# kkromberg/SpeechRecognition

Measured on AMD Instinct MI355X. Metric: frames/sec scored+decoded, higher is better.
Workload: dtype f64

## Files before the change

speechrecognition_amd/build.py:

```python
from __future__ import annotations

import hashlib
import os
import subprocess
import sys

HERE = os.path.dirname(os.path.abspath(__file__))
CSRC = os.path.join(HERE, "csrc")
LIB = os.path.join(HERE, "libsrgpu.so")
SOURCES = ["srgpu_api.cpp", "mixset.cpp", "feeder.cpp", "gmm_mfma.hip", "gmm_exact.hip", "gmm_prefilter.hip", "viterbi_decode.hip",
           "viterbi_fast.hip", "viterbi_words.hip", "viterbi_align.hip", "viterbi_fb.hip", "viterbi_netfb.hip", "viterbi_mmi.hip", "viterbi_smbr.hip", "viterbi_lattice.hip", "viterbi_bigram.hip", "viterbi_bigram_fb.hip", "viterbi_bigram_mmi.hip", "viterbi_bigram_lattice.hip",
           "em_accumulate.hip", "em_finalize.hip", "fmllr_stats.hip", "fmllr.cpp"]
HEADERS = ["kernels.h", "host_util.h", "handles.h", "traceback.h", "dpp_util.h", "netfb_device.h", os.path.join("..", "..", "include", "srgpu.h")]
FLAGS = ["-O3", "-std=c++17", "--offload-arch=gfx950", "-fPIC", "-fvisibility=hidden", "-Wall", "-Wno-unused-function"]
PER_FILE = {"gmm_exact.hip": ["-ffp-contract=off"], "gmm_prefilter.hip": ["-ffp-contract=off"], "em_accumulate.hip": ["-ffp-contract=off"],
            "em_finalize.hip": ["-ffp-contract=off"],
            "viterbi_bigram_lattice.hip": ["-ffp-contract=off"],
            "fmllr_stats.hip": ["-ffp-contract=off"]}
MAX_PARALLEL = 8


def _read(path):
    with open(path, "rb") as f:
        return f.read()


def _stamp_of(parts):
    h = hashlib.sha256()
    for p in parts:
        h.update(len(p).to_bytes(8, "little"))
        h.update(p)
    return h.hexdigest()


def _stored(path):
    try:
# ... 102 lines not shown
```

speechrecognition_amd/csrc/gmm_prefilter.hip:

```cpp
#include <hip/hip_runtime.h>
#include <stdint.h>

#include <algorithm>
#include <cmath>
#include <vector>

#include "kernels.h"

#ifndef SR_P16_NB
#define SR_P16_NB 4
#endif

namespace srgpu {

typedef float v4f __attribute__((ext_vector_type(4)));
static constexpr int kPWaves = 4;
static constexpr int kGroupBlocks = 8;

typedef _Float16 f16x8 __attribute__((ext_vector_type(8)));

__device__ inline uint32_t pack_f16x2(_Float16 l, _Float16 h) {
  return (uint32_t)__builtin_bit_cast(uint16_t, l) | ((uint32_t)__builtin_bit_cast(uint16_t, h) << 16);
}

template <int KS32, int NB>
__global__ __launch_bounds__(kPWaves * 64, (NB <= 2 ? 3 : 2)) void gmm_prefilter16_kernel(GmmPrefilterArgs a) {
  constexpr int kBlockBytes = KS32 * 1024;
  constexpr int kStageBytes = kGroupBlocks * kBlockBytes;
  constexpr int kChunksPerStage = kStageBytes / 1024;
  constexpr int kDmaPerWave = kChunksPerStage / kPWaves;
// ... 284 lines not shown
    case 4: hipLaunchKernelGGL((gmm_prefilter16_kernel<4, SR_P16_NB>), grid, block, 0, stream, a); break;
    default: return hipErrorInvalidValue;
  }
  return hipGetLastError();
}
int gmm_prefilter_frames_per_tile() { return kPWaves * SR_P16_NB * 16; }

#pragma clang fp contract(off)

#ifndef SR_R_THREADS
#define SR_R_THREADS 768
#endif
#ifndef SR_R_BATCH
#define SR_R_BATCH 4
#endif
static constexpr int kRThreads = SR_R_THREADS;
static constexpr int kRThreadsWide = 512;
static constexpr int kRWaves = kRThreads / 64;
static constexpr int kRBatch = SR_R_BATCH;
#ifndef SR_R_BATCH_WIDE
#define SR_R_BATCH_WIDE 8
#endif
static constexpr int kRBatchWide = SR_R_BATCH_WIDE;
static constexpr uint32_t kRingEntries = 128;
static constexpr uint32_t kRingLists = 2 * 8 * kRingEntries;
static constexpr uint32_t kRingWave = 4 * kRingLists;
struct __attribute__((aligned(16))) RingEntry { uint32_t lf, mask; double score; };
struct __attribute__((packed, aligned(4))) RowPiece { float v[4]; };

template <int DT, int NS, int SPW, int CH, int NT = kRThreads, int VS = 1, bool DEFER = false>
__global__ __launch_bounds__(NT) void gmm_refine_kernel(GmmRefineArgs a) {
  static_assert(DT > 0 && (DT & 1), "padded dimension: odd");
  static_assert(!DEFER || CH > 1, "deferred lists: states of several chunks");
  constexpr int kRThreads = NT, kRWaves = NT / 64;
  static_assert(CH == 1 || CH == 2 || CH == 4, "chunks per state (half)");
  static_assert(VS == 1 || (VS == 2 && CH == 4), "two halves only of four-chunk states");
  static_assert(SPW % (CH * VS) == 0 && (CH == 1 || SPW % 4 == 0), "a state's chunks live in one workgroup");
  extern __shared__ __attribute__((aligned(1024))) unsigned char panel_raw[];
  const uint32_t D = (uint32_t)DT, tid = threadIdx.x;
  const int lane = tid & 63, wave = tid >> 6;
  const uint32_t s0 = blockIdx.x * SPW;
  const uint32_t ns = (s0 + SPW <= a.n_pstates) ? SPW : a.n_pstates - s0;
  const uint32_t state_bytes = (2u * D + 2u) * NS * 8u;
  const uint64_t f_begin = (uint64_t)blockIdx.y * a.frames_per_split;
  const uint64_t f_end = (f_begin + a.frames_per_split < a.n_frames) ? f_begin + a.frames_per_split : a.n_frames;

  {
    const uint32_t chunks = (ns * state_bytes + 1023u) >> 10;
    const unsigned char* src = reinterpret_cast<const unsigned char*>(a.rows) + (uint64_t)s0 * state_bytes + lane * 16;
    for (uint32_t ch = wave; ch < chunks; ch += kRWaves)
// ... 10 lines not shown
  uint32_t n_eval = 0;
  double x[DT];
  const __amdgpu_buffer_rsrc_t featsT_rsrc = __builtin_amdgcn_make_buffer_rsrc(
      const_cast<float*>(a.featsT), 0, (int)0xFFFFFFFFu, 0x00020000);
  const uint32_t ld4 = (uint32_t)a.n_frames_ld * 4u;
  auto load_x = [&](uint64_t f) __attribute__((always_inline)) {
    const uint32_t voff = (uint32_t)f * 4u;
#pragma unroll
    for (int k = 0; k < DT; k++)
      x[k] = (double)__builtin_bit_cast(float, __builtin_amdgcn_raw_buffer_load_b32(featsT_rsrc, voff, (uint32_t)k * ld4, 0));
  };
  auto load_x_row = [&](uint64_t f) __attribute__((always_inline)) {
    const float* xr = a.feats + f * (uint64_t)DT;
#pragma unroll
    for (int q = 0; q < DT / 4; q++) {
      const RowPiece t = reinterpret_cast<const RowPiece*>(xr)[q];
#pragma unroll
      for (int i = 0; i < 4; i++) x[4 * q + i] = (double)t.v[i];
    }
#pragma unroll
    for (int k = DT - DT % 4; k < DT; k++) x[k] = (double)xr[k];
  };
  auto evaluate = [&](const unsigned char* col0) __attribute__((always_inline)) -> double {
    const volatile __attribute__((address_space(3))) double* col =
        (const volatile __attribute__((address_space(3))) double*)col0;
    double l0 = 0.0, l1 = 0.0, dist, score;
    {
      constexpr int RB = NT == kRThreadsWide ? kRBatchWide : kRBatch;
      constexpr int NB_ = (DT + 1 + RB - 1) / RB;
      double pm[2][RB], pv[2][RB];
#pragma unroll
      for (int i = 0; i < RB; i++)
        if (i <= DT) { pm[0][i] = col[(2 * i) * NS]; pv[0][i] = col[(2 * i + 1) * NS]; }
#pragma unroll
      for (int b = 0; b < NB_; b++) {
        const int cur = b & 1;
        __builtin_amdgcn_sched_barrier(0);
#pragma unroll
        for (int i = 0; i < RB; i++) {
          const int k = (b + 1) * RB + i;
          if (k <= DT) { pm[cur ^ 1][i] = col[(2 * k) * NS]; pv[cur ^ 1][i] = col[(2 * k + 1) * NS]; }
        }
        __builtin_amdgcn_sched_barrier(0);
#pragma unroll
        for (int i = 0; i < RB; i++) {
          const int k = b * RB + i;
          if (k < (int)(DT - (DT & 1))) {
            double u = x[k] - pm[cur][i];
            u = u * u;
            u = u * pv[cur][i];
            if (k & 1) l1 = l1 + u; else l0 = l0 + u;
          } else if (k == DT - 1) {
            dist = l0 + l1;
            const double t = x[k] - pm[cur][i];
            dist += t * t * pv[cur][i];
          } else if (k == DT) {
            if (!(DT & 1)) dist = l0 + l1;
            score = pm[cur][i] + dist / 2;
            score -= pv[cur][i];
          }
        }
        asm volatile("" : "+v"(l0), "+v"(l1));
      }
    }
// ... 22 lines not shown

  const uint32_t n_it = (uint32_t)((f_end - f_begin + kRThreads - 1) / kRThreads);
  for (uint32_t it = 0; it < n_it; it++) {
    const uint64_t fr = f_wave + (uint64_t)it * kRThreads + lane;
    const bool valid = fr < f_end;
    const uint64_t f = valid ? fr : f_end - 1;
    const uint32_t lf = it * 64u + (uint32_t)lane;
    load_x(f);
    constexpr int RS = SPW / (CH * VS);
    double res[RS];
    if constexpr (CH == 1) {
#pragma unroll
      for (int h = 0; h < SPW / 4; h++) {
        const uint4 v = reinterpret_cast<const uint4*>(a.mask)[(uint64_t)((s0 >> 2) + h) * a.n_frames + f];
        const uint32_t mk[4] = {v.x, v.y, v.z, v.w};
#pragma unroll
        for (int jj = 0; jj < 4; jj++) {
          const int j = 4 * h + jj;
          const uint32_t n = nd[j];
          uint32_t mask = mk[jj];
          mask &= n >= 32 ? 0xFFFFFFFFu : ((1u << n) - 1u);
          res[j] = 1e10;
          if (n) {
            const double score = evaluate(panel_raw + (size_t)j * state_bytes + (uint32_t)__builtin_ctz(mask | 0x80000000u) * 8u);
            res[j] = mask != 0 ? seeded_min(score) : res[j];
            if (counting) n_eval += (uint32_t)__builtin_popcountll(__ballot(valid));
          }
          const bool more = valid && (mask & (mask - 1)) != 0;
          const uint64_t b = __ballot(more);
          if (b) {
            const uint32_t c1 = (uint32_t)(cnt1 >> (8 * j)) & 0xFFu;
            const uint32_t pos = c1 + __builtin_amdgcn_mbcnt_hi((uint32_t)(b >> 32), __builtin_amdgcn_mbcnt_lo((uint32_t)b, 0u));
            if (more) {
              ring[(uint32_t)j * kRingEntries + pos] = RingEntry{lf, mask & (mask - 1), res[j]};
            }
            cnt1 += (uint64_t)__builtin_popcountll(b) << (8 * j);
          }
        }
      }
      if (valid) {
        if (a.chunks == 1) {
          double* o = a.out + f * a.ld + s0;
          if (ns == SPW) {
#pragma unroll
            for (int j = 0; j < SPW; j += 2) *reinterpret_cast<double2*>(o + j) = make_double2(res[j], res[j + 1]);
          } else {
#pragma unroll
// ... 12 lines not shown
#pragma unroll
          for (int j = 0; j < SPW; j += 4) {
            double m = res[j + 1] < res[j] ? res[j + 1] : res[j];
            m = res[j + 2] < m ? res[j + 2] : m;
            m = res[j + 3] < m ? res[j + 3] : m;
            if ((uint32_t)j < ns) o[j / 4] = m;
          }
        }
      }
    } else {
      auto append = [&](int j, bool more, uint32_t rest, double& best) __attribute__((always_inline)) {
        const uint64_t b = __ballot(more);
        if (b) {
          if constexpr (DEFER) {
            const uint32_t nb = (uint32_t)__builtin_popcountll(b);
            if (dcnt[DEFER ? j : 0] + nb <= a.defer_cap) {
              const uint32_t pos = dcnt[DEFER ? j : 0] + __builtin_amdgcn_mbcnt_hi((uint32_t)(b >> 32), __builtin_amdgcn_mbcnt_lo((uint32_t)b, 0u));
              if (more) seg[(uint64_t)j * a.defer_cap + pos] = RingEntry{(uint32_t)f, rest, best};
              dcnt[DEFER ? j : 0] += nb;
            } else {
              uint32_t mm = more ? rest : 0u;
              const unsigned char* panel = panel_raw + (size_t)j * state_bytes;
              do {
                const double score = evaluate(panel + (uint32_t)__builtin_ctz(mm | 0x80000000u) * 8u);
                if (counting) n_eval += (uint32_t)__builtin_popcountll(__ballot(mm != 0));
                if (mm != 0 && score < best) best = score;
                mm &= mm - 1;
              } while (__any(mm != 0));
            }
          } else {
          const uint32_t c1 = (uint32_t)(cnt1 >> (8 * j)) & 0xFFu;
          const uint32_t pos = c1 + __builtin_amdgcn_mbcnt_hi((uint32_t)(b >> 32), __builtin_amdgcn_mbcnt_lo((uint32_t)b, 0u));
          if (more) {
            ring[(uint32_t)j * kRingEntries + pos] = RingEntry{lf, rest, best};
          }
          cnt1 += (uint64_t)__builtin_popcountll(b) << (8 * j);
          }
        }
      };
      uint32_t mk[SPW];
#pragma unroll
      for (int h = 0; h < SPW / 4; h++) {
        const uint4 v = reinterpret_cast<const uint4*>(a.mask)[(uint64_t)((s0 >> 2) + h) * a.n_frames + f];
        mk[4 * h] = v.x; mk[4 * h + 1] = v.y; mk[4 * h + 2] = v.z; mk[4 * h + 3] = v.w;
      }
#pragma unroll
      for (int j = 0; j < SPW; j++) mk[j] &= nd[j] >= 32 ? 0xFFFFFFFFu : ((1u << nd[j]) - 1u);
      if constexpr (VS == 1) {
#pragma unroll
      for (int r = 0; r < RS; r++) {
        uint32_t msel = mk[r * CH], off = 0;
#pragma unroll
        for (int c = 1; c < CH; c++) {
          const bool empty = msel == 0;
          msel = empty ? mk[r * CH + c] : msel;
          off = empty ? (uint32_t)c * state_bytes : off;
        }
        res[r] = 1e10;
        if (nd[r * CH]) {
          const double score = evaluate(panel_raw + (size_t)(r * CH) * state_bytes + off + (uint32_t)__builtin_ctz(msel | 0x80000000u) * 8u);
          res[r] = msel != 0 ? seeded_min(score) : res[r];
          if (counting) n_eval += (uint32_t)__builtin_popcountll(__ballot(valid));
        }
#pragma unroll
        for (int c = 0; c < CH; c++) {
          const bool is_sel = off == (uint32_t)c * state_bytes;
          const uint32_t rest = is_sel ? msel & (msel - 1) : mk[r * CH + c];
          if (nd[r * CH + c]) append(r * CH + c, valid && rest != 0, rest, res[r]);
        }
      }
      } else {
#pragma unroll
      for (int r = 0; r < RS; r++) res[r] = 1e10;
#pragma unroll
      for (int rv = 0; rv < RS * VS; rv++) {
        uint32_t msel = mk[rv * CH], off = 0;
#pragma unroll
        for (int c = 1; c < CH; c++) {
          const bool empty = msel == 0;
          msel = empty ? mk[rv * CH + c] : msel;
          off = empty ? (uint32_t)c * state_bytes : off;
        }
        double resv = 1e10;
        if (nd[rv * CH]) {
          const double score = evaluate(panel_raw + (size_t)(rv * CH) * state_bytes + off + (uint32_t)__builtin_ctz(msel | 0x80000000u) * 8u);
          resv = msel != 0 ? seeded_min(score) : resv;
          if (counting) n_eval += (uint32_t)__builtin_popcountll(__ballot(valid));
        }
        if constexpr (VS == 1) res[rv] = resv;
        else res[rv / VS] = resv < res[rv / VS] ? resv : res[rv / VS];
#pragma unroll
        for (int c = 0; c < CH; c++) {
          const bool is_sel = off == (uint32_t)c * state_bytes;
          const uint32_t rest = is_sel ? msel & (msel - 1) : mk[rv * CH + c];
          if (nd[rv * CH + c]) append(rv * CH + c, valid && rest != 0, rest, resv);
        }
        if constexpr (DEFER && VS == 2) res[rv / VS] = resv < res[rv / VS] ? resv : res[rv / VS];
      }
      }
      if (valid) {
        double* o = a.out + f * a.ld + s0 / (CH * VS);
        if (ns == SPW && RS >= 2) {
#pragma unroll
          for (int r = 0; r + 1 < RS; r += 2) *reinterpret_cast<double2*>(o + r) = make_double2(res[r], res[r + 1]);
        } else {
#pragma unroll
          for (int r = 0; r < RS; r++)
            if ((uint32_t)(r * CH * VS) < ns) o[r] = res[r];
// ... 19 lines not shown
      const bool l1 = level == 1;
      const uint32_t have = (uint32_t)((l1 ? cnt1 : cnt2) >> (8u * j)) & 0xFFu;
      const uint32_t slot0 = ((level - 1u) * 8u + j) * kRingEntries;
      if (l1) cnt1 -= (uint64_t)n << (8u * j); else cnt2 -= (uint64_t)n << (8u * j);
      const bool live = (uint32_t)lane < n;
      asm volatile("" ::: "memory");
      __builtin_amdgcn_fence(__ATOMIC_RELEASE, "wavefront");
      __builtin_amdgcn_fence(__ATOMIC_ACQUIRE, "wavefront");
      asm volatile("" ::: "memory");
      const uint32_t at = slot0 + have - n + (live ? (uint32_t)lane : 0u);
      const RingEntry en = ring[at];
      const uint32_t lfb = en.lf;
      uint32_t m = live ? en.mask : 0u;
      double cur = en.score;
      const uint64_t fb = frame_of(lfb);
      load_x_row(fb);
      double* o = a.out + fb * a.ld + ((s0 + j) >> chunk_shift);
      if constexpr (CH == 1) {
        if (chunk_shift) cur = *o;
      }
      const double before = cur;
      const unsigned char* panel = panel_raw + (size_t)j * state_bytes;
      do {
        const double score = evaluate(panel + (uint32_t)__builtin_ctz(m | 0x80000000u) * 8u);
        if (counting) n_eval += (uint32_t)__builtin_popcountll(__ballot(m != 0));
        if (m != 0 && score < cur) cur = score;
        m &= m - 1;
      } while (!l1 && __any(m != 0));
      if (l1) {
        const uint64_t b = __ballot(m != 0);
        if (b) {
          const uint32_t c2 = (uint32_t)(cnt2 >> (8u * j)) & 0xFFu;
          const uint32_t pos = c2 + __builtin_amdgcn_mbcnt_hi((uint32_t)(b >> 32), __builtin_amdgcn_mbcnt_lo((uint32_t)b, 0u));
          if (m != 0) {
            ring[(8u + j) * kRingEntries + pos] = RingEntry{lfb, m, cur};
          }
          cnt2 += (uint64_t)__builtin_popcountll(b) << (8u * j);
        }
      }
      asm volatile("" ::: "memory");
      const bool lower = live && cur < before;
      if constexpr (CH == 1) {
        if (lower) *o = cur;
      } else {
        __builtin_amdgcn_fence(__ATOMIC_RELEASE, "wavefront");
        if (lower) (void)__builtin_amdgcn_global_atomic_fmin_f64((__attribute__((address_space(1))) double*)o, cur);
      }
// ... 32 lines not shown
  uint32_t nj[SPW];
#pragma unroll
  for (int j = 0; j < SPW; j++) nj[j] = (uint32_t)j < ns ? (uint32_t)__builtin_amdgcn_readfirstlane((int)a.defer_cnt[wave_global * SPW + j]) : 0u;
  __builtin_amdgcn_s_waitcnt(0x0F70);
  __syncthreads();
  const bool counting = a.n_refined != nullptr;
  uint32_t n_eval = 0;
  constexpr uint32_t chunk_shift = CH == 2 ? 1u : VS == 2 ? 3u : 2u;
  uint64_t cnt2 = 0;

  float xf[DT];
  auto load_row = [&](uint64_t f) __attribute__((always_inline)) {
    const float* xr = a.feats + f * (uint64_t)DT;
#pragma unroll
    for (int q = 0; q < DT / 4; q++) {
      const RowPiece t = reinterpret_cast<const RowPiece*>(xr)[q];
#pragma unroll
      for (int i = 0; i < 4; i++) xf[4 * q + i] = t.v[i];
    }
#pragma unroll
    for (int k = DT - DT % 4; k < DT; k++) xf[k] = xr[k];
  };
  auto evaluate = [&](const unsigned char* col0) __attribute__((always_inline)) -> double {
    const volatile __attribute__((address_space(3))) double* col = (const volatile __attribute__((address_space(3))) double*)col0;
    double l0 = 0.0, l1 = 0.0, dist, score;
    constexpr int NB_ = (DT + 1 + RB - 1) / RB;
    double pm[2][RB], pv[2][RB];
#pragma unroll
    for (int i = 0; i < RB; i++)
      if (i <= DT) { pm[0][i] = col[(2 * i) * NS]; pv[0][i] = col[(2 * i + 1) * NS]; }
#pragma unroll
    for (int b = 0; b < NB_; b++) {
      const int cur = b & 1;
      __builtin_amdgcn_sched_barrier(0);
#pragma unroll
      for (int i = 0; i < RB; i++) {
        const int k = (b + 1) * RB + i;
        if (k <= DT) { pm[cur ^ 1][i] = col[(2 * k) * NS]; pv[cur ^ 1][i] = col[(2 * k + 1) * NS]; }
      }
      __builtin_amdgcn_sched_barrier(0);
#pragma unroll
      for (int i = 0; i < RB; i++) {
        const int k = b * RB + i;
        if (k < DT - 1) {
          double u = (double)xf[k < DT ? k : 0] - pm[cur][i];
          u = u * u;
          u = u * pv[cur][i];
          if (k & 1) l1 = l1 + u; else l0 = l0 + u;
        } else if (k == DT - 1) {
          dist = l0 + l1;
          const double t = (double)xf[k < DT ? k : 0] - pm[cur][i];
          dist += t * t * pv[cur][i];
        } else if (k == DT) {
          score = pm[cur][i] + dist / 2;
          score -= pv[cur][i];
        }
      }
      asm volatile("" : "+v"(l0), "+v"(l1));
    }
    return score;
  };
  auto batch = [&](const bool l1, const uint32_t j, const RingEntry en, const bool live) __attribute__((always_inline)) {
    uint32_t m = live ? en.mask : 0u;
    double cur = en.score;
    const uint64_t fb = en.lf;
    load_row(fb);
    double* o = a.out + fb * a.ld + ((s0 + j) >> chunk_shift);
    const double before = cur;
    const unsigned char* panel = panel_raw + (size_t)j * state_bytes;
    do {
      const double score = evaluate(panel + (uint32_t)__builtin_ctz(m | 0x80000000u) * 8u);
      if (counting) n_eval += (uint32_t)__builtin_popcountll(__ballot(m != 0));
      if (m != 0 && score < cur) cur = score;
      m &= m - 1;
    } while (!l1 && __any(m != 0));
    if (l1) {
      const uint64_t b = __ballot(m != 0);
      if (b) {
        const uint32_t c2 = (uint32_t)(cnt2 >> (8u * j)) & 0xFFu;
        const uint32_t pos = c2 + __builtin_amdgcn_mbcnt_hi((uint32_t)(b >> 32), __builtin_amdgcn_mbcnt_lo((uint32_t)b, 0u));
        if (m != 0) ring[j * kRingEntries + pos] = RingEntry{en.lf, m, cur};
        cnt2 += (uint64_t)__builtin_popcountll(b) << (8u * j);
      }
    }
    if (live && cur < before) (void)__builtin_amdgcn_global_atomic_fmin_f64((__attribute__((address_space(1))) double*)o, cur);
  };
  auto level2 = [&](const bool flush) __attribute__((always_inline)) {
    for (;;) {
      const uint64_t pick = (cnt2 & 0x4040404040404040ull) ? (cnt2 & 0x4040404040404040ull) : flush ? cnt2 : 0ull;
      if (!pick) break;
      uint32_t j = (uint32_t)__builtin_ctzll(pick) >> 3;
      asm volatile("" : "+s"(j));
      const uint32_t have = (uint32_t)(cnt2 >> (8u * j)) & 0xFFu, n = have < 64u ? have : 64u;
      cnt2 -= (uint64_t)n << (8u * j);
// ... 56 lines not shown
    __syncthreads();
  }
}

hipError_t launch_transpose_feats(const float* feats, uint64_t n_frames, uint32_t dim, uint32_t dp, uint64_t ldT, float* out, float* featsP,
                                  hipStream_t stream) {
  if (n_frames == 0) return hipSuccess;
  if (dp < dim || (dp != dim && !featsP)) return hipErrorInvalidValue;
  hipLaunchKernelGGL(transpose_feats_kernel, dim3((unsigned)((n_frames + 63) / 64)), dim3(256), 0, stream, feats, n_frames, dim, dp, ldT, out,
                     dp != dim ? featsP : nullptr);
  return hipGetLastError();
}

int gmm_refine_slots(uint32_t max_dens, uint32_t padded_dim) { return padded_dim > 39 ? 32 : max_dens <= 8 ? 8 : max_dens <= 16 ? 16 : 32; }

uint32_t gmm_refine_padded_dim(uint32_t dim) {
  static const uint32_t bounds[] = {9, 17, 25, 33, 39, 47, 55, 63};
  const uint32_t need = dim | 1u;
  for (uint32_t b : bounds)
    if (need <= b) return b;
  return 0;
}

static int refine_threads(uint32_t dp) { return dp <= 47 ? kRThreads : kRThreadsWide; }
static int refine_spw(const GmmRefineArgs& a) {
  return (size_t)(2 * a.dim + 2) * a.n_slots * 8 * 8 <= 160 * 1024 ? 8 : 4;
}
static void refine_grid(const GmmRefineArgs& a, int spw, uint32_t* n_sgroups, uint64_t* splits, uint64_t* frames_per_split) {
  const uint64_t nt = (uint64_t)refine_threads(a.dim);
  *n_sgroups = (a.n_pstates + spw - 1) / spw;
  uint64_t sp = std::max<uint64_t>(1, (512 + *n_sgroups - 1) / *n_sgroups);
  sp = std::min<uint64_t>(sp, (a.n_frames + nt - 1) / nt);
  sp = std::max<uint64_t>(sp, 1);
  *frames_per_split = (a.n_frames + sp - 1) / sp;
  *splits = *frames_per_split ? (a.n_frames + *frames_per_split - 1) / *frames_per_split : 1;
}
size_t gmm_refine_ring_words(const GmmRefineArgs& a) {
  uint32_t g; uint64_t sp, fps;
  refine_grid(a, refine_spw(a), &g, &sp, &fps);
  return (size_t)g * sp * kRWaves * kRingWave;
}

static uint32_t defer_cap_for(const GmmRefineArgs& a, int spw) {
  uint32_t g; uint64_t sp, fps;
  refine_grid(a, spw, &g, &sp, &fps);
  const uint64_t per_wave = ((fps + kRThreads - 1) / kRThreads) * 64;
  return (uint32_t)std::min<uint64_t>(((per_wave / 4 + 63) & ~(uint64_t)63) + 64, 1u << 30);
}
void gmm_refine_defer_layout(const GmmRefineArgs& a, size_t budget_bytes, uint32_t cap_limit, uint32_t* cap, size_t* n_entries,
                             size_t* n_counts) {
  *cap = 0; *n_entries = 0; *n_counts = 0;
  if (a.chunks < 2 || a.dim > 39 || a.n_slots != 32 || a.n_frames == 0) return;
  uint32_t g; uint64_t sp, fps;
  refine_grid(a, 8, &g, &sp, &fps);
  uint32_t c = defer_cap_for(a, 8);
  if (cap_limit) c = std::min(c, cap_limit);
  const size_t segs = (size_t)g * sp * kRWaves * 8;
  if (segs * c * 16 > budget_bytes) return;
  *cap = c; *n_entries = segs * c; *n_counts = segs;
}

template <int DT, int NS, int SPW, int CH, int NT, int VS = 1>
static hipError_t launch_refine_one(const GmmRefineArgs& a0, hipStream_t stream) {
  GmmRefineArgs a = a0;
  const size_t state_bytes = (size_t)(2 * DT + 2) * NS * 8;
  const size_t smem = (SPW * state_bytes + 1023) & ~(size_t)1023;
  uint32_t n_sgroups;
  uint64_t splits;
  refine_grid(a, SPW, &n_sgroups, &splits, &a.frames_per_split);
  const dim3 grid(n_sgroups, (unsigned)splits), block(NT);
  if constexpr (CH > 1 && NT == kRThreads && SPW == 8) {
    if (a.defer && a.defer_cnt && a.defer_cap) {
      auto k1 = gmm_refine_kernel<DT, NS, SPW, CH, NT, VS, true>;
      auto k2 = gmm_drain_kernel<DT, NS, SPW, CH, NT, VS>;
      hipError_t e = hipFuncSetAttribute((const void*)k1, hipFuncAttributeMaxDynamicSharedMemorySize, (int)smem);
      if (e == hipSuccess) e = hipFuncSetAttribute((const void*)k2, hipFuncAttributeMaxDynamicSharedMemorySize, (int)smem);
      if (e != hipSuccess) return e;
      hipLaunchKernelGGL(k1, grid, block, smem, stream, a);
      if ((e = hipGetLastError()) != hipSuccess) return e;
      hipLaunchKernelGGL(k2, grid, block, smem, stream, a);
      return hipGetLastError();
    }
  }
  a.defer = nullptr; a.defer_cnt = nullptr; a.defer_cap = 0;
  auto kernel = gmm_refine_kernel<DT, NS, SPW, CH, NT, VS>;
  hipError_t e = hipFuncSetAttribute((const void*)kernel, hipFuncAttributeMaxDynamicSharedMemorySize, (int)smem);
  if (e != hipSuccess) return e;
  hipLaunchKernelGGL(kernel, grid, block, smem, stream, a);
  return hipGetLastError();
}

template <int DT>
static hipError_t launch_refine_narrow(const GmmRefineArgs& a, hipStream_t stream) {
  switch (a.n_slots) {
    case 8: return launch_refine_one<DT, 8, 8, 1, kRThreads>(a, stream);
    case 16: return launch_refine_one<DT, 16, 8, 1, kRThreads>(a, stream);
    case 32:
      if (a.chunks == 2) return launch_refine_one<DT, 32, 8, 2, kRThreads>(a, stream);
      if (a.chunks == 4) return launch_refine_one<DT, 32, 8, 4, kRThreads>(a, stream);
      if (a.chunks == 8) return launch_refine_one<DT, 32, 8, 4, kRThreads, 2>(a, stream);
      return launch_refine_one<DT, 32, 8, 1, kRThreads>(a, stream);
    default: return hipErrorInvalidValue;
  }
}
template <int DT>
static hipError_t launch_refine_wide(const GmmRefineArgs& a, hipStream_t stream) {
  if (a.n_slots != 32) return hipErrorInvalidValue;
  if (a.chunks == 2) return launch_refine_one<DT, 32, 4, 2, kRThreadsWide>(a, stream);
  if (a.chunks == 4) return launch_refine_one<DT, 32, 4, 4, kRThreadsWide>(a, stream);
  return launch_refine_one<DT, 32, 4, 1, kRThreadsWide>(a, stream);
}

hipError_t launch_gmm_refine(const GmmRefineArgs& a, hipStream_t stream) {
  if (a.n_frames == 0) return hipSuccess;
  if (!a.ring || (uint64_t)a.dim * a.n_frames_ld * 4u >= (1ull << 32)) return hipErrorInvalidValue;
  if (a.chunks != 1 && (a.n_slots != 32 || (a.chunks != 2 && a.chunks != 4 && a.chunks != 8))) return hipErrorInvalidValue;
  if (a.chunks == 8 && a.dim > 39) return hipErrorInvalidValue;
  switch (a.dim) {
    case 9: return launch_refine_narrow<9>(a, stream);
    case 17: return launch_refine_narrow<17>(a, stream);
    case 25: return launch_refine_narrow<25>(a, stream);
    case 33: return launch_refine_narrow<33>(a, stream);
    case 39: return launch_refine_narrow<39>(a, stream);
    case 47:
      if (a.n_slots != 32) return hipErrorInvalidValue;
      return a.chunks == 2 ? launch_refine_one<47, 32, 4, 2, kRThreads>(a, stream) : a.chunks == 4 ? launch_refine_one<47, 32, 4, 4, kRThreads>(a, stream)
                           : launch_refine_one<47, 32, 4, 1, kRThreads>(a, stream);
    case 55: return launch_refine_wide<55>(a, stream);
    case 63: return launch_refine_wide<63>(a, stream);
    default: return hipErrorInvalidValue;
  }
}

}
```

speechrecognition_amd/csrc/handles.h:

```cpp
#pragma once
#include <hip/hip_runtime.h>

#include <atomic>
#include <condition_variable>
#include <cstdint>
#include <map>
#include <memory>
#include <mutex>
#include <string>
#include <thread>
#include <vector>

#include "../../include/srgpu.h"
#include "host_util.h"
#include "kernels.h"

namespace srhost {
int fail(int code, const char* fmt, ...) __attribute__((format(printf, 2, 3)));
}

#define HIP_TRY(expr)                                                                             \
  do {                                                                                            \
    hipError_t e_ = (expr);                                                                       \
    if (e_ != hipSuccess) return srhost::fail(SR_EHIP, "%s: %s (%s:%d)", #expr, hipGetErrorString(e_), __FILE__, __LINE__); \
// ... 49 lines not shown
  bool max_approx = true;
  DevBuf<uint32_t> dens_off;
  DevBuf<double> means, inv_vars, norm, logw;
  DevBuf<uint32_t> dens_mean, dens_var;
  std::vector<uint32_t> h_dens_off, h_dens_mean, h_dens_var;
  std::vector<double> h_means, h_inv_vars, h_norm, h_logw;
  bool mfma_packed = false, pf_packed = false;
  uint32_t n_mean = 0, n_var = 0;
  int ksteps = 0;
  uint32_t n_blocks = 0, n_groups = 0;
  DevBuf<double> apack;
  DevBuf<uint32_t> blk_meta, grp_state;
  std::vector<uint32_t> group_first_block;
  std::map<uint32_t, std::unique_ptr<DevBuf<uint32_t>>> split_tabs, pf_split_tabs;
  const uint32_t *split_cur = nullptr, *pf_split_cur = nullptr;
  uint32_t split_ny = 0;
  int pf_ks32 = 0;
  uint32_t pf_groups = 0, pf_ny = 0, max_dens = 0, pf_slots = 0, pf_chunks = 1, pf_pstates = 0;
  DevBuf<unsigned char> pf_apack;
  DevBuf<float> pf_lim, featsT, featsP;
  DevBuf<uint4> pf_defer;
  DevBuf<uint32_t> pf_defer_cnt;
  int neg_possible = -1;
  uint32_t pf_dp = 0;
  DevBuf<uint32_t> pf_mask, pf_ndens, pf_ring;
  DevBuf<double> pf_rows;
  DevBuf<unsigned long long> pf_counter;
  hipStream_t s_copy = nullptr;
  float* staging[2] = {nullptr, nullptr};
  hipEvent_t staging_free[2] = {nullptr, nullptr};
  std::atomic<bool> staging_busy{false};
  std::mutex spare_mu;
  std::unique_ptr<CorpusSpare> spare;
  std::vector<sr_corpus*> corpora;
  hipStream_t s_gmm = nullptr, s_search = nullptr;
  DevBuf<double> scores[2];
  hipEvent_t ev_scored[2] = {nullptr, nullptr}, ev_consumed[2] = {nullptr, nullptr};
  size_t chunk_frames = 0;
  bool overlap = true;
  size_t defer_budget = (size_t)32 << 30;
  uint32_t defer_cap_limit = 0;
  size_t fb_budget = (size_t)1 << 30;
  bool profiling = false;
  std::vector<EventPair> events;
  sr_profile prof{};
};
// ... 168 lines not shown
```

speechrecognition_amd/csrc/kernels.h:

```cpp
#pragma once
#include <hip/hip_runtime.h>
#include <stdint.h>

#include <vector>

namespace srgpu {

struct GmmMfmaArgs {
  const float* feats;
  uint64_t n_frames;
  uint32_t dim;
  const double* apack;
  const uint32_t* blk_meta;
  const uint32_t* grp_state;
  const uint32_t* split_begin;
  double* out;
  uint32_t ld;
  uint32_t nx, ny;
};
int gmm_mfma_ksteps_for_dim(uint32_t dim);
int gmm_mfma_frames_per_tile(int ksteps);
hipError_t launch_gmm_mfma(const GmmMfmaArgs& a, int ksteps, bool sum, hipStream_t stream);

struct GmmExactArgs {
// ... 35 lines not shown
  uint32_t chunks;
};
struct PfBound { float kappa, acc, abs, sub; };
constexpr float kPfRes16 = 4.8835e-4f;
inline constexpr PfBound pf_bound(int ks32) {
  return ks32 == 4 ? PfBound{1.05e-3f, 1.6e-5f, 7.0e-7f, 3.38e-7f} : PfBound{1.05e-3f, 1.1e-5f, 6.0e-7f, 2.92e-7f};
}
struct GmmRefineArgs {
  const float* feats;
  const float* featsT;
  uint64_t n_frames, n_frames_ld;
  uint32_t dim, n_pstates, chunks;
  const uint32_t* n_dens_ps;
  const double* rows;
  uint32_t n_slots;
  const uint32_t* mask;
  double* out; uint32_t ld;
  uint64_t frames_per_split;
  unsigned long long* n_refined;
  uint32_t* ring;
  void* defer;
  uint32_t* defer_cnt;
  uint32_t defer_cap;
};
void gmm_refine_defer_layout(const GmmRefineArgs& a, size_t budget_bytes, uint32_t cap_limit, uint32_t* cap, size_t* n_entries,
                             size_t* n_counts);
size_t gmm_refine_ring_words(const GmmRefineArgs& a);
hipError_t launch_gmm_prefilter(const GmmPrefilterArgs& a, int ks32, hipStream_t stream);
int gmm_prefilter_frames_per_tile();
hipError_t probe_fp16_denormals(hipStream_t stream, bool* preserved);
hipError_t probe_fp16_accumulation(hipStream_t stream, int ks32, bool* ok, double* worst_ratio);
uint32_t gmm_refine_padded_dim(uint32_t dim);
int gmm_refine_slots(uint32_t max_dens, uint32_t padded_dim);
hipError_t launch_gmm_refine(const GmmRefineArgs& a, hipStream_t stream);
hipError_t launch_transpose_feats(const float* feats, uint64_t n_frames, uint32_t dim, uint32_t dp, uint64_t ldT, float* out, float* featsP,
                                  hipStream_t stream);

struct DecodeNet {
  uint32_t n_slots;
  uint32_t n_words;
  const uint32_t* slot_info;
  const uint32_t* slot_word;
  const uint32_t* word_end_slot;
  uint32_t silence_word;
  double tdp_loop, tdp_forward, tdp_skip;
  uint32_t silence_state;
};
static constexpr uint32_t kSlotPos0 = 1u << 16;
static constexpr uint32_t kSlotPos1 = 1u << 17;
static constexpr uint32_t kSlotEnd = 1u << 18;
static constexpr uint32_t kSlotSilState = 1u << 19;
static constexpr uint32_t kSlotSilWord = 1u << 20;
static constexpr uint32_t kSlotFirstSil = 1u << 21;
static constexpr uint32_t kSlotSingle = 1u << 22;
struct FastNet {
  uint32_t n_slots;
  const uint32_t* state;
// ... 510 lines not shown
```

speechrecognition_amd/csrc/srgpu_api.cpp:

```cpp
#include <hip/hip_runtime.h>

#include <algorithm>
#include <cmath>
#include <cstdarg>
#include <cstdio>
#include <cstdlib>
#include <cstring>
#include <limits>
#include <map>
#include <memory>
#include <mutex>
#include <numeric>
#include <queue>
#include <set>
#include <string>
#include <vector>

#include "../../include/srgpu.h"
#include "host_util.h"
#include "kernels.h"
#include "traceback.h"

using namespace srgpu;
using srhost::guarded;
// ... 116 lines not shown
    return n > lo ? std::min(32u, n - lo) : 0u;
  };
  {
    std::vector<uint32_t> cnt(PS);
    for (uint32_t ps = 0; ps < PS; ps++) cnt[ps] = ps_count(ps);
    HIP_TRY(m->pf_ndens.upload(cnt.data(), cnt.size()));
  }
  {
    const uint32_t NS = (uint32_t)gmm_refine_slots(std::min(32u, m->max_dens), DP), planes = 2 * DP + 2;
    const uint32_t pairs = D - (D & 1u);
    auto slot_of = [&](uint32_t d) -> uint32_t { return d < pairs ? d : DP - 1u; };
    m->pf_slots = NS;
    const size_t n_rows_d = (size_t)PS * planes * NS + 128;
    std::unique_ptr<double[]> rows_own(new double[n_rows_d]);
    double* const rows_p = rows_own.get();
    std::fill(rows_p + (size_t)PS * planes * NS, rows_p + n_rows_d, 0.0);
    srhost::parallel_ranges(PS, 64, [&](size_t ps0, size_t ps1) {
    for (uint32_t ps = (uint32_t)ps0; ps < (uint32_t)ps1; ps++) {
      double* r = rows_p + (size_t)ps * planes * NS;
      std::fill(r, r + (size_t)planes * NS, 0.0);
      for (uint32_t i = 0; i < ps_count(ps); i++) {
        const size_t c = (size_t)dens_off[ps / Cs] + 32u * (ps % Cs) + i;
        const uint32_t sl = i;
        for (uint32_t d = 0; d < D; d++) { r[(2 * slot_of(d)) * NS + sl] = means[c * D + d]; r[(2 * slot_of(d) + 1) * NS + sl] = inv_vars[c * D + d]; }
        r[(2 * DP) * NS + sl] = norm[c];
        r[(2 * DP + 1) * NS + sl] = logw[c];
      }
    }
    });
    HIP_TRY(m->pf_rows.upload(rows_p, n_rows_d));
  }
  const uint32_t n_groups = (PS + 3) / 4;
  const float finf = std::numeric_limits<float>::infinity();
  auto coeffs = [&](size_t c, std::vector<double>& arow) -> double {
    double q2 = 0.0;
    for (uint32_t d = 0; d < D; d++) {
      const double mu = means[c * D + d], iv = inv_vars[c * D + d];
      arow[2 * d] = 0.5 * iv;
      arow[2 * d + 1] = -mu * iv;
      q2 += mu * mu * iv;
    }
    return norm[c] - logw[c] + 0.5 * q2;
  };
  double sA = 1.0;
  {
    std::mutex mu_big;
    double big = 0.0;
    srhost::parallel_ranges((size_t)m->n_dens, 4096, [&](size_t c0, size_t c1) {
      std::vector<double> arow(32 * (size_t)KS);
      double mine = 0.0;
      for (size_t c = c0; c < c1; c++) {
        const double konst = coeffs(c, arow);
        if (std::isfinite(konst)) mine = std::max(mine, std::fabs(konst));
// ... 134 lines not shown
  if (!m->profiling) return SR_OK;
  ep->kind = kind;
  HIP_TRY(hipEventCreate(&ep->a));
  HIP_TRY(hipEventCreate(&ep->b));
  HIP_TRY(hipEventRecord(ep->a, s));
  return SR_OK;
}
int prof_end(sr_model* m, hipStream_t s, EventPair* ep) {
  if (!m->profiling) return SR_OK;
  HIP_TRY(hipEventRecord(ep->b, s));
  m->events.push_back(*ep);
  return SR_OK;
}

int resolve_dense_kernel(const sr_model* m, int gmm_kernel) {
  if (gmm_kernel == SR_GMM_DEFAULT) gmm_kernel = m->max_approx ? SR_GMM_PREFILTER : SR_GMM_MFMA;
  if (gmm_kernel == SR_GMM_MFMA && m->ksteps == 0) gmm_kernel = SR_GMM_EXACT;
  return gmm_kernel;
}

GmmRefineArgs refine_shape(const sr_model* m, uint64_t n_frames) {
  GmmRefineArgs ra{};
  ra.n_frames = n_frames; ra.dim = m->pf_dp; ra.n_pstates = m->pf_pstates; ra.n_slots = m->pf_slots; ra.chunks = m->pf_chunks;
  return ra;
}
struct DeferLayout { uint32_t cap; size_t n_e, n_c; };
DeferLayout defer_layout(const sr_model* m, uint64_t n_frames) {
  DeferLayout d;
  gmm_refine_defer_layout(refine_shape(m, n_frames), m->defer_budget, m->defer_cap_limit, &d.cap, &d.n_e, &d.n_c);
  return d;
}

int reserve_scoring(sr_model* m, int gmm_kernel, uint64_t n_max) {
  gmm_kernel = resolve_dense_kernel(m, gmm_kernel);
  if ((gmm_kernel == SR_GMM_MFMA && !m->mfma_packed) || (gmm_kernel == SR_GMM_PREFILTER && !m->pf_packed)) {
    int rc = srhost::ensure_host_tables(m);
    if (rc) return rc;
  }
  if (gmm_kernel == SR_GMM_MFMA && !m->mfma_packed) {
    int rc = pack_model(m, m->h_dens_off.data(), m->h_means.data(), m->h_inv_vars.data(), m->h_norm.data(), m->h_logw.data());
    if (rc) return rc;
    m->mfma_packed = true;
  }
  if (gmm_kernel == SR_GMM_PREFILTER && !m->pf_packed) {
    int rc = pack_prefilter(m, m->h_dens_off.data(), m->h_means.data(), m->h_inv_vars.data(), m->h_norm.data(), m->h_logw.data());
    if (rc) return rc;
// ... 3643 lines not shown
```

Baseline: 13.81 million.

## Interleave mean/inv-var params and size refine splits by CU occupancy

Packs each dimension's mean and inverse variance next to each other in the refine row table so the kernel reads both with one 16-byte LDS load instead of two strided 8-byte loads. Separately, it replaces the fixed 512-block split heuristic with an occupancy-aware split count, computed from the CU count and the blocks-per-CU occupancy query, plus a per-split overhead term to balance work across rounds. The ring and defer sizing are moved into a shared header and now use the maximum wave count. This risks different tail balancing and larger workspace allocations.

```diff
diff --git a/speechrecognition_amd/build.py b/speechrecognition_amd/build.py
--- a/speechrecognition_amd/build.py
+++ b/speechrecognition_amd/build.py
@@ -11,7 +11,7 @@
 SOURCES = ["srgpu_api.cpp", "mixset.cpp", "feeder.cpp", "gmm_mfma.hip", "gmm_exact.hip", "gmm_prefilter.hip", "viterbi_decode.hip",
            "viterbi_fast.hip", "viterbi_words.hip", "viterbi_align.hip", "viterbi_fb.hip", "viterbi_netfb.hip", "viterbi_mmi.hip", "viterbi_smbr.hip", "viterbi_lattice.hip", "viterbi_bigram.hip", "viterbi_bigram_fb.hip", "viterbi_bigram_mmi.hip", "viterbi_bigram_lattice.hip",
            "em_accumulate.hip", "em_finalize.hip", "fmllr_stats.hip", "fmllr.cpp"]
-HEADERS = ["kernels.h", "host_util.h", "handles.h", "traceback.h", "dpp_util.h", "netfb_device.h", os.path.join("..", "..", "include", "srgpu.h")]
+HEADERS = ["kernels.h", "host_util.h", "handles.h", "traceback.h", "dpp_util.h", "netfb_device.h", "refine_split.h", os.path.join("..", "..", "include", "srgpu.h")]
 FLAGS = ["-O3", "-std=c++17", "--offload-arch=gfx950", "-fPIC", "-fvisibility=hidden", "-Wall", "-Wno-unused-function"]
 PER_FILE = {"gmm_exact.hip": ["-ffp-contract=off"], "gmm_prefilter.hip": ["-ffp-contract=off"], "em_accumulate.hip": ["-ffp-contract=off"],
             "em_finalize.hip": ["-ffp-contract=off"],
diff --git a/speechrecognition_amd/csrc/gmm_prefilter.hip b/speechrecognition_amd/csrc/gmm_prefilter.hip
--- a/speechrecognition_amd/csrc/gmm_prefilter.hip
+++ b/speechrecognition_amd/csrc/gmm_prefilter.hip
@@ -6,6 +6,7 @@
 #include <vector>
 
 #include "kernels.h"
+#include "refine_split.h"
 
 #ifndef SR_P16_NB
 #define SR_P16_NB 4
@@ -336,10 +337,9 @@
 #define SR_R_BATCH_WIDE 8
 #endif
 static constexpr int kRBatchWide = SR_R_BATCH_WIDE;
-static constexpr uint32_t kRingEntries = 128;
-static constexpr uint32_t kRingLists = 2 * 8 * kRingEntries;
-static constexpr uint32_t kRingWave = 4 * kRingLists;
+static_assert(kRWaves <= (int)kRefineWavesMax, "the list workspace is sized for 768 threads");
 struct __attribute__((aligned(16))) RingEntry { uint32_t lf, mask; double score; };
+typedef double ParamPair __attribute__((ext_vector_type(2)));
 struct __attribute__((packed, aligned(4))) RowPiece { float v[4]; };
 
 template <int DT, int NS, int SPW, int CH, int NT = kRThreads, int VS = 1, bool DEFER = false>
@@ -396,8 +396,8 @@
     for (int k = DT - DT % 4; k < DT; k++) x[k] = (double)xr[k];
   };
   auto evaluate = [&](const unsigned char* col0) __attribute__((always_inline)) -> double {
-    const volatile __attribute__((address_space(3))) double* col =
-        (const volatile __attribute__((address_space(3))) double*)col0;
+    const volatile __attribute__((address_space(3))) ParamPair* col =
+        (const volatile __attribute__((address_space(3))) ParamPair*)col0;
     double l0 = 0.0, l1 = 0.0, dist, score;
     {
       constexpr int RB = NT == kRThreadsWide ? kRBatchWide : kRBatch;
@@ -405,7 +405,7 @@
       double pm[2][RB], pv[2][RB];
 #pragma unroll
       for (int i = 0; i < RB; i++)
-        if (i <= DT) { pm[0][i] = col[(2 * i) * NS]; pv[0][i] = col[(2 * i + 1) * NS]; }
+        if (i <= DT) { const ParamPair t = col[i * NS]; pm[0][i] = t.x; pv[0][i] = t.y; }
 #pragma unroll
       for (int b = 0; b < NB_; b++) {
         const int cur = b & 1;
@@ -413,7 +413,7 @@
 #pragma unroll
         for (int i = 0; i < RB; i++) {
           const int k = (b + 1) * RB + i;
-          if (k <= DT) { pm[cur ^ 1][i] = col[(2 * k) * NS]; pv[cur ^ 1][i] = col[(2 * k + 1) * NS]; }
+          if (k <= DT) { const ParamPair t = col[k * NS]; pm[cur ^ 1][i] = t.x; pv[cur ^ 1][i] = t.y; }
         }
         __builtin_amdgcn_sched_barrier(0);
 #pragma unroll
@@ -482,7 +482,7 @@
           mask &= n >= 32 ? 0xFFFFFFFFu : ((1u << n) - 1u);
           res[j] = 1e10;
           if (n) {
-            const double score = evaluate(panel_raw + (size_t)j * state_bytes + (uint32_t)__builtin_ctz(mask | 0x80000000u) * 8u);
+            const double score = evaluate(panel_raw + (size_t)j * state_bytes + (uint32_t)__builtin_ctz(mask | 0x80000000u) * 16u);
             res[j] = mask != 0 ? seeded_min(score) : res[j];
             if (counting) n_eval += (uint32_t)__builtin_popcountll(__ballot(valid));
           }
@@ -541,7 +541,7 @@
               uint32_t mm = more ? rest : 0u;
               const unsigned char* panel = panel_raw + (size_t)j * state_bytes;
               do {
-                const double score = evaluate(panel + (uint32_t)__builtin_ctz(mm | 0x80000000u) * 8u);
+                const double score = evaluate(panel + (uint32_t)__builtin_ctz(mm | 0x80000000u) * 16u);
                 if (counting) n_eval += (uint32_t)__builtin_popcountll(__ballot(mm != 0));
                 if (mm != 0 && score < best) best = score;
                 mm &= mm - 1;
@@ -577,7 +577,7 @@
         }
         res[r] = 1e10;
         if (nd[r * CH]) {
-          const double score = evaluate(panel_raw + (size_t)(r * CH) * state_bytes + off + (uint32_t)__builtin_ctz(msel | 0x80000000u) * 8u);
+          const double score = evaluate(panel_raw + (size_t)(r * CH) * state_bytes + off + (uint32_t)__builtin_ctz(msel | 0x80000000u) * 16u);
           res[r] = msel != 0 ? seeded_min(score) : res[r];
           if (counting) n_eval += (uint32_t)__builtin_popcountll(__ballot(valid));
         }
@@ -602,7 +602,7 @@
         }
         double resv = 1e10;
         if (nd[rv * CH]) {
-          const double score = evaluate(panel_raw + (size_t)(rv * CH) * state_bytes + off + (uint32_t)__builtin_ctz(msel | 0x80000000u) * 8u);
+          const double score = evaluate(panel_raw + (size_t)(rv * CH) * state_bytes + off + (uint32_t)__builtin_ctz(msel | 0x80000000u) * 16u);
           resv = msel != 0 ? seeded_min(score) : resv;
           if (counting) n_eval += (uint32_t)__builtin_popcountll(__ballot(valid));
         }
@@ -668,7 +668,7 @@
       const double before = cur;
       const unsigned char* panel = panel_raw + (size_t)j * state_bytes;
       do {
-        const double score = evaluate(panel + (uint32_t)__builtin_ctz(m | 0x80000000u) * 8u);
+        const double score = evaluate(panel + (uint32_t)__builtin_ctz(m | 0x80000000u) * 16u);
         if (counting) n_eval += (uint32_t)__builtin_popcountll(__ballot(m != 0));
         if (m != 0 && score < cur) cur = score;
         m &= m - 1;
@@ -747,13 +747,13 @@
     for (int k = DT - DT % 4; k < DT; k++) xf[k] = xr[k];
   };
   auto evaluate = [&](const unsigned char* col0) __attribute__((always_inline)) -> double {
-    const volatile __attribute__((address_space(3))) double* col = (const volatile __attribute__((address_space(3))) double*)col0;
+    const volatile __attribute__((address_space(3))) ParamPair* col = (const volatile __attribute__((address_space(3))) ParamPair*)col0;
     double l0 = 0.0, l1 = 0.0, dist, score;
     constexpr int NB_ = (DT + 1 + RB - 1) / RB;
     double pm[2][RB], pv[2][RB];
 #pragma unroll
     for (int i = 0; i < RB; i++)
-      if (i <= DT) { pm[0][i] = col[(2 * i) * NS]; pv[0][i] = col[(2 * i + 1) * NS]; }
+      if (i <= DT) { const ParamPair t = col[i * NS]; pm[0][i] = t.x; pv[0][i] = t.y; }
 #pragma unroll
     for (int b = 0; b < NB_; b++) {
       const int cur = b & 1;
@@ -761,7 +761,7 @@
 #pragma unroll
       for (int i = 0; i < RB; i++) {
         const int k = (b + 1) * RB + i;
-        if (k <= DT) { pm[cur ^ 1][i] = col[(2 * k) * NS]; pv[cur ^ 1][i] = col[(2 * k + 1) * NS]; }
+        if (k <= DT) { const ParamPair t = col[k * NS]; pm[cur ^ 1][i] = t.x; pv[cur ^ 1][i] = t.y; }
       }
       __builtin_amdgcn_sched_barrier(0);
 #pragma unroll
@@ -794,7 +794,7 @@
     const double before = cur;
     const unsigned char* panel = panel_raw + (size_t)j * state_bytes;
     do {
-      const double score = evaluate(panel + (uint32_t)__builtin_ctz(m | 0x80000000u) * 8u);
+      const double score = evaluate(panel + (uint32_t)__builtin_ctz(m | 0x80000000u) * 16u);
       if (counting) n_eval += (uint32_t)__builtin_popcountll(__ballot(m != 0));
       if (m != 0 && score < cur) cur = score;
       m &= m - 1;
@@ -897,53 +897,27 @@
   return 0;
 }
 
-static int refine_threads(uint32_t dp) { return dp <= 47 ? kRThreads : kRThreadsWide; }
-static int refine_spw(const GmmRefineArgs& a) {
-  return (size_t)(2 * a.dim + 2) * a.n_slots * 8 * 8 <= 160 * 1024 ? 8 : 4;
-}
-static void refine_grid(const GmmRefineArgs& a, int spw, uint32_t* n_sgroups, uint64_t* splits, uint64_t* frames_per_split) {
-  const uint64_t nt = (uint64_t)refine_threads(a.dim);
-  *n_sgroups = (a.n_pstates + spw - 1) / spw;
-  uint64_t sp = std::max<uint64_t>(1, (512 + *n_sgroups - 1) / *n_sgroups);
-  sp = std::min<uint64_t>(sp, (a.n_frames + nt - 1) / nt);
-  sp = std::max<uint64_t>(sp, 1);
-  *frames_per_split = (a.n_frames + sp - 1) / sp;
-  *splits = *frames_per_split ? (a.n_frames + *frames_per_split - 1) / *frames_per_split : 1;
-}
-size_t gmm_refine_ring_words(const GmmRefineArgs& a) {
-  uint32_t g; uint64_t sp, fps;
-  refine_grid(a, refine_spw(a), &g, &sp, &fps);
-  return (size_t)g * sp * kRWaves * kRingWave;
-}
-
-static uint32_t defer_cap_for(const GmmRefineArgs& a, int spw) {
-  uint32_t g; uint64_t sp, fps;
-  refine_grid(a, spw, &g, &sp, &fps);
-  const uint64_t per_wave = ((fps + kRThreads - 1) / kRThreads) * 64;
-  return (uint32_t)std::min<uint64_t>(((per_wave / 4 + 63) & ~(uint64_t)63) + 64, 1u << 30);
-}
+static RefineShape shape_of(const GmmRefineArgs& a) { return RefineShape{a.n_frames, a.dim, a.n_pstates, a.n_slots, a.chunks, a.cu_slots}; }
+size_t gmm_refine_ring_words(const GmmRefineArgs& a) { return refine_ring_words_for(shape_of(a)); }
 void gmm_refine_defer_layout(const GmmRefineArgs& a, size_t budget_bytes, uint32_t cap_limit, uint32_t* cap, size_t* n_entries,
                              size_t* n_counts) {
-  *cap = 0; *n_entries = 0; *n_counts = 0;
-  if (a.chunks < 2 || a.dim > 39 || a.n_slots != 32 || a.n_frames == 0) return;
-  uint32_t g; uint64_t sp, fps;
-  refine_grid(a, 8, &g, &sp, &fps);
-  uint32_t c = defer_cap_for(a, 8);
-  if (cap_limit) c = std::min(c, cap_limit);
-  const size_t segs = (size_t)g * sp * kRWaves * 8;
-  if (segs * c * 16 > budget_bytes) return;
-  *cap = c; *n_entries = segs * c; *n_counts = segs;
+  refine_defer_layout_for(shape_of(a), budget_bytes, cap_limit, cap, n_entries, n_counts);
 }
 
 template <int DT, int NS, int SPW, int CH, int NT, int VS = 1>
-static hipError_t launch_refine_one(const GmmRefineArgs& a0, hipStream_t stream) {
+static hipError_t launch_refine_one(const GmmRefineArgs& a0, hipStream_t stream, int* occ) {
   GmmRefineArgs a = a0;
   const size_t state_bytes = (size_t)(2 * DT + 2) * NS * 8;
   const size_t smem = (SPW * state_bytes + 1023) & ~(size_t)1023;
-  uint32_t n_sgroups;
-  uint64_t splits;
-  refine_grid(a, SPW, &n_sgroups, &splits, &a.frames_per_split);
-  const dim3 grid(n_sgroups, (unsigned)splits), block(NT);
+  if (occ) {
+    auto kernel = gmm_refine_kernel<DT, NS, SPW, CH, NT, VS>;
+    hipError_t e = hipFuncSetAttribute((const void*)kernel, hipFuncAttributeMaxDynamicSharedMemorySize, (int)smem);
+    if (e != hipSuccess) return e;
+    return hipOccupancyMaxActiveBlocksPerMultiprocessor(occ, (const void*)kernel, NT, smem);
+  }
+  const RefineGrid g = refine_grid_for(shape_of(a), SPW);
+  a.frames_per_split = g.splits.long_len;
+  const dim3 grid(g.n_sgroups, g.splits.n_splits), block(NT);
   if constexpr (CH > 1 && NT == kRThreads && SPW == 8) {
     if (a.defer && a.defer_cnt && a.defer_cap) {
       auto k1 = gmm_refine_kernel<DT, NS, SPW, CH, NT, VS, true>;
@@ -966,45 +940,53 @@
 }
 
 template <int DT>
-static hipError_t launch_refine_narrow(const GmmRefineArgs& a, hipStream_t stream) {
+static hipError_t launch_refine_narrow(const GmmRefineArgs& a, hipStream_t stream, int* occ) {
   switch (a.n_slots) {
-    case 8: return launch_refine_one<DT, 8, 8, 1, kRThreads>(a, stream);
-    case 16: return launch_refine_one<DT, 16, 8, 1, kRThreads>(a, stream);
+    case 8: return launch_refine_one<DT, 8, 8, 1, kRThreads>(a, stream, occ);
+    case 16: return launch_refine_one<DT, 16, 8, 1, kRThreads>(a, stream, occ);
     case 32:
-      if (a.chunks == 2) return launch_refine_one<DT, 32, 8, 2, kRThreads>(a, stream);
-      if (a.chunks == 4) return launch_refine_one<DT, 32, 8, 4, kRThreads>(a, stream);
-      if (a.chunks == 8) return launch_refine_one<DT, 32, 8, 4, kRThreads, 2>(a, stream);
-      return launch_refine_one<DT, 32, 8, 1, kRThreads>(a, stream);
+      if (a.chunks == 2) return launch_refine_one<DT, 32, 8, 2, kRThreads>(a, stream, occ);
+      if (a.chunks == 4) return launch_refine_one<DT, 32, 8, 4, kRThreads>(a, stream, occ);
+      if (a.chunks == 8) return launch_refine_one<DT, 32, 8, 4, kRThreads, 2>(a, stream, occ);
+      return launch_refine_one<DT, 32, 8, 1, kRThreads>(a, stream, occ);
     default: return hipErrorInvalidValue;
   }
 }
 template <int DT>
-static hipError_t launch_refine_wide(const GmmRefineArgs& a, hipStream_t stream) {
+static hipError_t launch_refine_wide(const GmmRefineArgs& a, hipStream_t stream, int* occ) {
   if (a.n_slots != 32) return hipErrorInvalidValue;
-  if (a.chunks == 2) return launch_refine_one<DT, 32, 4, 2, kRThreadsWide>(a, stream);
-  if (a.chunks == 4) return launch_refine_one<DT, 32, 4, 4, kRThreadsWide>(a, stream);
-  return launch_refine_one<DT, 32, 4, 1, kRThreadsWide>(a, stream);
+  if (a.chunks == 2) return launch_refine_one<DT, 32, 4, 2, kRThreadsWide>(a, stream, occ);
+  if (a.chunks == 4) return launch_refine_one<DT, 32, 4, 4, kRThreadsWide>(a, stream, occ);
+  return launch_refine_one<DT, 32, 4, 1, kRThreadsWide>(a, stream, occ);
+}
+
+static hipError_t refine_dispatch(const GmmRefineArgs& a, hipStream_t stream, int* occ) {
+  if (a.chunks != 1 && (a.n_slots != 32 || (a.chunks != 2 && a.chunks != 4 && a.chunks != 8))) return hipErrorInvalidValue;
+  if (a.chunks == 8 && a.dim > 39) return hipErrorInvalidValue;
+  switch (a.dim) {
+    case 9: return launch_refine_narrow<9>(a, stream, occ);
+    case 17: return launch_refine_narrow<17>(a, stream, occ);
+    case 25: return launch_refine_narrow<25>(a, stream, occ);
+    case 33: return launch_refine_narrow<33>(a, stream, occ);
+    case 39: return launch_refine_narrow<39>(a, stream, occ);
+    case 47:
+      if (a.n_slots != 32) return hipErrorInvalidValue;
+      return a.chunks == 2 ? launch_refine_one<47, 32, 4, 2, kRThreads>(a, stream, occ) : a.chunks == 4 ? launch_refine_one<47, 32, 4, 4, kRThreads>(a, stream, occ)
+                           : launch_refine_one<47, 32, 4, 1, kRThreads>(a, stream, occ);
+    case 55: return launch_refine_wide<55>(a, stream, occ);
+    case 63: return launch_refine_wide<63>(a, stream, occ);
+    default: return hipErrorInvalidValue;
+  }
 }
 
 hipError_t launch_gmm_refine(const GmmRefineArgs& a, hipStream_t stream) {
   if (a.n_frames == 0) return hipSuccess;
   if (!a.ring || (uint64_t)a.dim * a.n_frames_ld * 4u >= (1ull << 32)) return hipErrorInvalidValue;
-  if (a.chunks != 1 && (a.n_slots != 32 || (a.chunks != 2 && a.chunks != 4 && a.chunks != 8))) return hipErrorInvalidValue;
-  if (a.chunks == 8 && a.dim > 39) return hipErrorInvalidValue;
-  switch (a.dim) {
-    case 9: return launch_refine_narrow<9>(a, stream);
-    case 17: return launch_refine_narrow<17>(a, stream);
-    case 25: return launch_refine_narrow<25>(a, stream);
-    case 33: return launch_refine_narrow<33>(a, stream);
-    case 39: return launch_refine_narrow<39>(a, stream);
-    case 47:
-      if (a.n_slots != 32) return hipErrorInvalidValue;
-      return a.chunks == 2 ? launch_refine_one<47, 32, 4, 2, kRThreads>(a, stream) : a.chunks == 4 ? launch_refine_one<47, 32, 4, 4, kRThreads>(a, stream)
-                           : launch_refine_one<47, 32, 4, 1, kRThreads>(a, stream);
-    case 55: return launch_refine_wide<55>(a, stream);
-    case 63: return launch_refine_wide<63>(a, stream);
-    default: return hipErrorInvalidValue;
-  }
-}
-
-}
+  return refine_dispatch(a, stream, nullptr);
+}
+hipError_t gmm_refine_blocks_per_cu(const GmmRefineArgs& a, int* blocks) {
+  *blocks = 0;
+  return refine_dispatch(a, nullptr, blocks);
+}
+
+}
diff --git a/speechrecognition_amd/csrc/handles.h b/speechrecognition_amd/csrc/handles.h
--- a/speechrecognition_amd/csrc/handles.h
+++ b/speechrecognition_amd/csrc/handles.h
@@ -95,6 +95,7 @@
   DevBuf<uint4> pf_defer;
   DevBuf<uint32_t> pf_defer_cnt;
   int neg_possible = -1;
+  uint32_t pf_cu_slots = 0;
   uint32_t pf_dp = 0;
   DevBuf<uint32_t> pf_mask, pf_ndens, pf_ring;
   DevBuf<double> pf_rows;
diff --git a/speechrecognition_amd/csrc/kernels.h b/speechrecognition_amd/csrc/kernels.h
--- a/speechrecognition_amd/csrc/kernels.h
+++ b/speechrecognition_amd/csrc/kernels.h
@@ -81,6 +81,7 @@
   void* defer;
   uint32_t* defer_cnt;
   uint32_t defer_cap;
+  uint32_t cu_slots;
 };
 void gmm_refine_defer_layout(const GmmRefineArgs& a, size_t budget_bytes, uint32_t cap_limit, uint32_t* cap, size_t* n_entries,
                              size_t* n_counts);
@@ -92,6 +93,7 @@
 uint32_t gmm_refine_padded_dim(uint32_t dim);
 int gmm_refine_slots(uint32_t max_dens, uint32_t padded_dim);
 hipError_t launch_gmm_refine(const GmmRefineArgs& a, hipStream_t stream);
+hipError_t gmm_refine_blocks_per_cu(const GmmRefineArgs& a, int* blocks);
 hipError_t launch_transpose_feats(const float* feats, uint64_t n_frames, uint32_t dim, uint32_t dp, uint64_t ldT, float* out, float* featsP,
                                   hipStream_t stream);
 
diff --git a/speechrecognition_amd/csrc/refine_split.h b/speechrecognition_amd/csrc/refine_split.h
--- /dev/null
+++ b/speechrecognition_amd/csrc/refine_split.h
@@ -0,0 +1,87 @@
+#pragma once
+#include <algorithm>
+#include <cstddef>
+#include <cstdint>
+
+namespace srgpu {
+
+constexpr uint32_t kRingEntries = 128;
+constexpr uint32_t kRingLists = 2 * 8 * kRingEntries;
+constexpr uint32_t kRingWave = 4 * kRingLists;
+constexpr uint32_t kRefineWavesMax = 12;
+
+#ifndef SR_R_SPLIT_OVERHEAD
+#define SR_R_SPLIT_OVERHEAD 6
+#endif
+constexpr uint64_t kRefineSplitOverhead = SR_R_SPLIT_OVERHEAD;
+
+struct RefineSplits {
+  uint64_t long_len;
+  uint32_t n_long;
+  uint32_t n_splits;
+};
+
+inline RefineSplits refine_splits(uint32_t n_groups, uint32_t cu_slots, uint64_t n_frames, uint32_t n_threads) {
+  const uint64_t G = std::max<uint32_t>(1, n_groups), slots = std::max<uint32_t>(1, cu_slots), T = std::max<uint32_t>(1, n_threads);
+  if (n_frames == 0) return RefineSplits{0, 0, 1};
+  const uint64_t passes = (n_frames + T - 1) / T;
+  const uint64_t want = std::max<uint64_t>(1, (2 * slots + G - 1) / G);
+  uint64_t L;
+  if (want >= passes) {
+    const uint64_t sp = std::max<uint64_t>(1, std::min(want, passes));
+    L = ((passes + sp - 1) / sp) * T;
+  } else {
+    const uint64_t rounds = (G * want + slots - 1) / slots;
+    const uint64_t work = G * n_frames + G * kRefineSplitOverhead * T;
+    L = (work + rounds * slots - 1) / (rounds * slots);
+    L = std::min<uint64_t>(((L + T - 1) / T) * T, passes * T);
+  }
+  RefineSplits s;
+  s.long_len = L;
+  s.n_long = (uint32_t)(n_frames / L);
+  s.n_splits = s.n_long + (n_frames % L ? 1u : 0u);
+  return s;
+}
+
+struct RefineShape {
+  uint64_t n_frames;
+  uint32_t dim, n_pstates, n_slots, chunks;
+  uint32_t cu_slots;
+};
+struct RefineGrid { uint32_t n_sgroups; RefineSplits splits; };
+
+#ifndef SR_R_THREADS
+#define SR_R_THREADS 768
+#endif
+inline uint32_t refine_threads_for(uint32_t dp) { return dp <= 47 ? (uint32_t)SR_R_THREADS : 512u; }
+inline uint32_t refine_spw_for(uint32_t dp, uint32_t n_slots) { return (size_t)(2 * dp + 2) * n_slots * 8 * 8 <= 160 * 1024 ? 8u : 4u; }
+inline RefineGrid refine_grid_for(const RefineShape& a, uint32_t spw) {
+  RefineGrid g;
+  g.n_sgroups = (a.n_pstates + spw - 1) / spw;
+  g.splits = refine_splits(g.n_sgroups, a.cu_slots ? a.cu_slots : 256u, a.n_frames, refine_threads_for(a.dim));
+  return g;
+}
+inline size_t refine_ring_words_for(const RefineShape& a) {
+  const RefineGrid g = refine_grid_for(a, refine_spw_for(a.dim, a.n_slots));
+  return (size_t)g.n_sgroups * g.splits.n_splits * kRefineWavesMax * kRingWave;
+}
+inline uint32_t refine_defer_cap_for(const RefineShape& a, uint32_t spw) {
+  const RefineGrid g = refine_grid_for(a, spw);
+  const uint64_t T = refine_threads_for(a.dim);
+  const uint64_t longest = g.splits.n_long ? g.splits.long_len : a.n_frames;
+  const uint64_t per_wave = ((longest + T - 1) / T) * 64;
+  return (uint32_t)std::min<uint64_t>(((per_wave / 4 + 63) & ~(uint64_t)63) + 64, 1u << 30);
+}
+inline void refine_defer_layout_for(const RefineShape& a, size_t budget_bytes, uint32_t cap_limit, uint32_t* cap, size_t* n_entries,
+                                    size_t* n_counts) {
+  *cap = 0; *n_entries = 0; *n_counts = 0;
+  if (a.chunks < 2 || a.dim > 39 || a.n_slots != 32 || a.n_frames == 0) return;
+  const RefineGrid g = refine_grid_for(a, 8);
+  uint32_t c = refine_defer_cap_for(a, 8);
+  if (cap_limit) c = std::min(c, cap_limit);
+  const size_t segs = (size_t)g.n_sgroups * g.splits.n_splits * kRefineWavesMax * 8;
+  if (segs * c * 16 > budget_bytes) return;
+  *cap = c; *n_entries = segs * c; *n_counts = segs;
+}
+
+}
diff --git a/speechrecognition_amd/csrc/srgpu_api.cpp b/speechrecognition_amd/csrc/srgpu_api.cpp
--- a/speechrecognition_amd/csrc/srgpu_api.cpp
+++ b/speechrecognition_amd/csrc/srgpu_api.cpp
@@ -162,13 +162,21 @@
       for (uint32_t i = 0; i < ps_count(ps); i++) {
         const size_t c = (size_t)dens_off[ps / Cs] + 32u * (ps % Cs) + i;
         const uint32_t sl = i;
-        for (uint32_t d = 0; d < D; d++) { r[(2 * slot_of(d)) * NS + sl] = means[c * D + d]; r[(2 * slot_of(d) + 1) * NS + sl] = inv_vars[c * D + d]; }
-        r[(2 * DP) * NS + sl] = norm[c];
-        r[(2 * DP + 1) * NS + sl] = logw[c];
+        for (uint32_t d = 0; d < D; d++) { double* q = r + ((size_t)slot_of(d) * NS + sl) * 2; q[0] = means[c * D + d]; q[1] = inv_vars[c * D + d]; }
+        double* q = r + ((size_t)DP * NS + sl) * 2;
+        q[0] = norm[c];
+        q[1] = logw[c];
       }
     }
     });
     HIP_TRY(m->pf_rows.upload(rows_p, n_rows_d));
+    hipDeviceProp_t prop;
+    HIP_TRY(hipGetDeviceProperties(&prop, m->device));
+    GmmRefineArgs shape{};
+    shape.dim = DP; shape.n_slots = NS; shape.chunks = Cs;
+    int per_cu = 0;
+    if (gmm_refine_blocks_per_cu(shape, &per_cu) != hipSuccess) { (void)hipGetLastError(); per_cu = 1; }
+    m->pf_cu_slots = (uint32_t)std::max(1, prop.multiProcessorCount) * (uint32_t)std::max(1, per_cu);
   }
   const uint32_t n_groups = (PS + 3) / 4;
   const float finf = std::numeric_limits<float>::infinity();
@@ -349,6 +357,7 @@
 GmmRefineArgs refine_shape(const sr_model* m, uint64_t n_frames) {
   GmmRefineArgs ra{};
   ra.n_frames = n_frames; ra.dim = m->pf_dp; ra.n_pstates = m->pf_pstates; ra.n_slots = m->pf_slots; ra.chunks = m->pf_chunks;
+  ra.cu_slots = m->pf_cu_slots;
   return ra;
 }
 struct DeferLayout { uint32_t cap; size_t n_e, n_c; };
```

Result: slower. 13.46 million (-2.5%).
